# cbrl/BNN-PYNQ

Measured on AMD Instinct MI355X. Metric: images/sec (whole node) CNV-W1A1 CIFAR-10-shape batch, higher is better.
Workload: dtype u1; 1 GPU; cnvW1A1, 131072 synthetic 32x32x3 uint8 images per GPU per step, inputs resident in HBM, params cifar10/cnvW1A1; parallelism=dp1 (batch shards, no data-path collective)

## Files before the change

### bnn-pynq_amd/csrc/kernels.hip

```cpp
#include <hip/hip_runtime.h>
#include <hip/hip_ext.h>
#include <stdint.h>

#include <cstdlib>
#include <cstring>
#include <type_traits>

#define BNN_HD __host__ __device__
#include "act_faults.h"
#include "kernels.h"
#include "packed_params.h"
static_assert(bnn::kL0TileOffset == (int)bnn::kL0MfmaTileOffset && bnn::kL0BigBytes == (int)bnn::kL0MfmaBigBytes,
              "k_conv0_tile's operand offsets must be the ones packed_params.cpp writes the layer-0 table by");

namespace bnn {
namespace {

typedef const uint32_t __attribute__((address_space(4))) *kptr32;
typedef const uint64_t __attribute__((address_space(4))) *kptr64;

constexpr int kBlock = 256;
constexpr int kLfcFusedMaxA2 = 2048;

struct BlockMap { int cg, item; bool valid; };
// ... 410 lines not shown
      const uint4 v = wt[(tap * 2 + mt) * 64 + lane];
      wreg[tap][mt] = v8i{(int)v.x, (int)v.y, (int)v.z, (int)v.w, 0, 0, 0, 0};
    }
  __shared__ v16f seed_lds[2][2];
  if (tid < 64) reinterpret_cast<float *>(seed_lds)[tid] = reinterpret_cast<const float *>(tab + kL1MfmaWeights)[tid];
  const int cc = c < 28 ? c : 27;
  uint32_t pre[15];
  auto fetch = [&](int pair) {
    const int img0 = pair * 2, lim = min(2, n_images - img0) * 1800;
#pragma unroll
    for (int j = 0; j < 15; j++) {
      const int d = tid + 256 * j;
      pre[j] = d < lim ? in[(size_t)img0 * 1800 + d] : 0u;
    }
  };
  if (blockIdx.x * 2 < n_images) fetch(blockIdx.x);
  for (int pair = blockIdx.x; pair * 2 < n_images; pair += gridDim.x) {
    const int img0 = pair * 2, nimg = min(2, n_images - img0);
    __syncthreads();
#pragma unroll
    for (int j = 0; j < 15; j++) {
      const int d = tid + 256 * j;
      if (d < nimg * 1800) {
        const int i = d >= 1800, e = d - i * 1800, pix = e >> 1, hh = e & 1;
        const uint32_t bits = pre[j];
        plane[i][hh][pix] = make_uint4(lut[bits & 255], lut[(bits >> 8) & 255], lut[(bits >> 16) & 255], lut[bits >> 24]);
      }
    }
    if ((pair + gridDim.x) * 2 < n_images) fetch(pair + gridDim.x);
    __syncthreads();
    for (int rp = wave; rp < nimg * 14; rp += 4) {
      const int i = rp / 14, r = rp - i * 14;
      const uint4 *__restrict__ P = &plane[i][h][0];
      v16f acc[2][2] = {{seed_lds[0][h], seed_lds[0][h]}, {seed_lds[1][h], seed_lds[1][h]}};
#pragma unroll
      for (int kx = 0; kx < 3; kx++) {
        v8i b[4];
#pragma unroll
        for (int y = 0; y < 4; y++) {
          const uint4 v = P[(2 * r + y) * 30 + cc + kx];
          b[y] = v8i{(int)v.x, (int)v.y, (int)v.z, (int)v.w, 0, 0, 0, 0};
        }
#pragma unroll
        for (int ky = 0; ky < 3; ky++)
#pragma unroll
          for (int mt = 0; mt < 2; mt++)
#pragma unroll
            for (int pt = 0; pt < 2; pt++)
              acc[mt][pt] = __builtin_amdgcn_mfma_scale_f32_32x32x64_f8f6f4(wreg[ky * 3 + kx][mt], b[ky + pt], acc[mt][pt], 4, 4, 0,
                                                                              0x7F7F7F7F, 0, 0x7F7F7F7F);
      }
      uint32_t word[2];
#pragma unroll
      for (int mt = 0; mt < 2; mt++) {
        int v[16];
#pragma unroll
        for (int k = 0; k < 16; k++) v[k] = __float_as_int(fmaxf(acc[mt][0][k], acc[mt][1][k]));
        const uint32_t nf = or_halves(sign_nibbles(v, h));
        const uint32_t pooled = nf & (uint32_t)__builtin_amdgcn_mov_dpp((int)nf, 0xB1, 0xF, 0xF, true);
        word[mt] = ~pooled;
      }
      if (h == 0 && c < 28 && !(c & 1))
        *reinterpret_cast<uint2 *>(out + ((size_t)(img0 + i) * 196 + r * 14 + (c >> 1)) * 2) = make_uint2(word[0], word[1]);
    }
  }
}

template <int WIN, int CD, int NT, bool POOL, int G>
__global__ __launch_bounds__(256, 2) void k_conv_mfma(const uint32_t *__restrict__ in, uint32_t *__restrict__ out,
                                                       const uint8_t *__restrict__ tab, int n_images) {
  constexpr int WOUT = WIN - 2, RP = WOUT / 2, IPI = RP * WOUT, KH = CD / 2, KS = 9 * KH, STREAMS = 4 / NT;
  constexpr int PIX = WIN * WIN, DWI = PIX * CD, NPF = (G * DWI + 255) / 256;
  static_assert(WOUT % 2 == 0 && IPI % 2 == 0 && (NT == 2 || NT == 4), "tile geometry");
  __shared__ uint4 plane[G][CD][PIX];
  __shared__ uint32_t lut[256];
  const int tid = threadIdx.x, lane = tid & 63, wave = tid >> 6, mt = wave % NT, c = lane & 31, h = lane >> 5;
  lut[tid] = fp4_pm1((uint32_t)tid);
  const uint4 *__restrict__ wt = reinterpret_cast<const uint4 *>(tab);
  v8i wreg[KS];
#pragma unroll
  for (int ks = 0; ks < KS; ks++) {
    const uint4 v = wt[(ks * NT + mt) * 64 + lane];
    wreg[ks] = v8i{(int)v.x, (int)v.y, (int)v.z, (int)v.w, 0, 0, 0, 0};
  }
  const v16f seed = reinterpret_cast<const v16f *>(tab + (size_t)KS * NT * 64 * 16)[mt * 2 + h];
  const int ngroups = (n_images + G - 1) / G;
  uint32_t pre[NPF];
  auto fetch = [&](int grp) {
    const int img0 = grp * G, lim = min(G, n_images - img0) * DWI;
#pragma unroll
    for (int j = 0; j < NPF; j++) {
      const int d = tid + 256 * j;
      pre[j] = d < lim ? in[(size_t)img0 * DWI + d] : 0u;
    }
  };
  if (blockIdx.x < ngroups) fetch(blockIdx.x);
  for (int grp = blockIdx.x; grp < ngroups; grp += gridDim.x) {
    const int img0 = grp * G, nimg = min(G, n_images - img0), nitems = nimg * IPI;
    __syncthreads();
#pragma unroll
    for (int j = 0; j < NPF; j++) {
      const int d = tid + 256 * j;
      if (d < nimg * DWI) {
        const int i = d / DWI, e = d - i * DWI, pix = e / CD, q = e % CD;
        const uint32_t bits = pre[j];
        plane[i][q][pix] = make_uint4(lut[bits & 255], lut[(bits >> 8) & 255], lut[(bits >> 16) & 255], lut[bits >> 24]);
      }
    }
    if (grp + (int)gridDim.x < ngroups) fetch(grp + gridDim.x);
    __syncthreads();
    for (int t0 = (wave / NT) * 32; t0 < nitems; t0 += 32 * STREAMS) {
      const int item = min(t0 + c, nitems - 1);
      const int i = item / IPI, rem = item - i * IPI, rp = rem / WOUT, x = rem - rp * WOUT;
      v16f acc[2] = {seed, seed};
#pragma unroll
      for (int kh = 0; kh < KH; kh++) {
        const uint4 *__restrict__ P = &plane[i][kh * 2 + h][2 * rp * WIN + x];
#pragma unroll
        for (int kx = 0; kx < 3; kx++) {
          v8i b[4];
#pragma unroll
          for (int y = 0; y < 4; y++) {
            const uint4 v = P[y * WIN + kx];
            b[y] = v8i{(int)v.x, (int)v.y, (int)v.z, (int)v.w, 0, 0, 0, 0};
          }
#pragma unroll
          for (int ky = 0; ky < 3; ky++)
#pragma unroll
            for (int dy = 0; dy < 2; dy++)
              acc[dy] = __builtin_amdgcn_mfma_scale_f32_32x32x64_f8f6f4(wreg[(ky * 3 + kx) * KH + kh], b[ky + dy], acc[dy], 4, 4, 0,
                                                                         0x7F7F7F7F, 0, 0x7F7F7F7F);
        }
      }
      const bool valid = t0 + c < nitems;
      const size_t img = (size_t)(img0 + i);
      if constexpr (POOL) {
        int v[16];
#pragma unroll
        for (int k = 0; k < 16; k++) v[k] = __float_as_int(fmaxf(acc[0][k], acc[1][k]));
        const uint32_t nf = or_halves(sign_nibbles(v, h));
        const uint32_t pooled = nf & (uint32_t)__builtin_amdgcn_mov_dpp((int)nf, 0xB1, 0xF, 0xF, true);
        if (valid && h == 0 && !(x & 1)) out[(img * (RP * RP) + rp * RP + (x >> 1)) * NT + mt] = ~pooled;
      } else {
        uint32_t nf[2];
#pragma unroll
        for (int dy = 0; dy < 2; dy++) {
          int v[16];
#pragma unroll
          for (int k = 0; k < 16; k++) v[k] = __float_as_int(acc[dy][k]);
          nf[dy] = or_halves(sign_nibbles(v, h));
        }
        if (valid) out[(img * (WOUT * WOUT) + (2 * rp + h) * WOUT + x) * NT + mt] = ~(h ? nf[1] : nf[0]);
      }
    }
  }
}

__global__ __launch_bounds__(256) void k_conv_mfma_table(const uint32_t *__restrict__ rows, int row_dw, int ksteps, int tiles,
                                                          int mw, uint8_t *__restrict__ dst) {
  const int idx = blockIdx.x * 256 + threadIdx.x, nw = ksteps * tiles * 64;
  if (idx < nw) {
    const int ks = idx / (tiles * 64), mt = (idx / 64) % tiles, lane = idx & 63, n = 32 * mt + (lane & 31), h = lane >> 5;
    const uint32_t bits = rows[(size_t)n * row_dw + 2 + 2 * ks + h];
    reinterpret_cast<uint4 *>(dst)[idx] = make_uint4(fp4_pm1(bits & 255), fp4_pm1((bits >> 8) & 255), fp4_pm1((bits >> 16) & 255),
                                                     fp4_pm1(bits >> 24));
  } else if (idx < nw + tiles * 32) {
    const int j = idx - nw, mt = j >> 5, h = (j >> 4) & 1, reg = j & 15;
    const int n = 32 * mt + (reg & 3) + 8 * (reg >> 2) + 4 * h;
    long long t = (int)rows[(size_t)n * row_dw];
    t = t < -1 ? -1 : (t > mw + 2 ? mw + 2 : t);
    reinterpret_cast<float *>(dst + (size_t)nw * 16)[j] = (float)(-(mw - 2 * t) - 1);
  }
}

__device__ __forceinline__ uint32_t nibble_spread(uint32_t byte) {
  uint32_t t = byte & 0xFFu;
  t = (t | (t << 12)) & 0x000F000Fu;
  t = (t | (t << 6)) & 0x03030303u;
  return (t | (t << 3)) & 0x11111111u;
}
__device__ __forceinline__ uint4 fp4_planes(const uint32_t *lutz, const uint32_t *luts, uint32_t sg, uint32_t nz) {
  const uint32_t m = sg & nz;
  return make_uint4(lutz[nz & 255] | luts[m & 255], lutz[(nz >> 8) & 255] | luts[(m >> 8) & 255],
                    lutz[(nz >> 16) & 255] | luts[(m >> 16) & 255], lutz[nz >> 24] | luts[m >> 24]);
}
__device__ __forceinline__ void not_fired(const v16f &acc, const v16f &dt, int h, uint32_t &n0, uint32_t &n1) {
  int v[16], u[16];
#pragma unroll
  for (int k = 0; k < 16; k++) {
    v[k] = __float_as_int(acc[k]);
    u[k] = __float_as_int(acc[k] - dt[k]);
  }
  n0 = or_halves(sign_nibbles(v, h));
  n1 = or_halves(sign_nibbles(u, h));
}

template <int WIN, int CD, int NT, bool POOL, int G>
__global__ __launch_bounds__(256, 2) void k_conv_mfma_a2(const uint4 *__restrict__ in, uint32_t *__restrict__ out,
                                                          const uint8_t *__restrict__ tab, int n_images) {
  constexpr int WOUT = WIN - 2, RP = WOUT / 2, IPI = RP * WOUT, KH = CD / 2, KS = 9 * KH, STREAMS = 4 / NT;
  constexpr int PIX = WIN * WIN, QWI = PIX * KH, NPF = (G * QWI + 255) / 256;
  static_assert(WOUT % 2 == 0 && IPI % 2 == 0 && (NT == 2 || NT == 4), "tile geometry");
  __shared__ uint4 plane[G][CD][PIX];
  __shared__ uint32_t lutz[256], luts[256];
  const int tid = threadIdx.x, lane = tid & 63, wave = tid >> 6, mt = wave % NT, c = lane & 31, h = lane >> 5;
  lutz[tid] = nibble_spread((uint32_t)tid) << 1;
  luts[tid] = nibble_spread((uint32_t)tid) << 3;
  const uint4 *__restrict__ wt = reinterpret_cast<const uint4 *>(tab);
  v8i wreg[KS];
#pragma unroll
  for (int ks = 0; ks < KS; ks++) {
    const uint4 v = wt[(ks * NT + mt) * 64 + lane];
    wreg[ks] = v8i{(int)v.x, (int)v.y, (int)v.z, (int)v.w, 0, 0, 0, 0};
  }
  const v16f *__restrict__ cst = reinterpret_cast<const v16f *>(tab + (size_t)KS * NT * 64 * 16);
  const v16f seed = cst[mt * 2 + h], dt = cst[NT * 2 + mt * 2 + h];
  const int ngroups = (n_images + G - 1) / G;
  uint4 pre[NPF];
  auto fetch = [&](int grp) {
    const int img0 = grp * G, lim = min(G, n_images - img0) * QWI;
#pragma unroll
    for (int j = 0; j < NPF; j++) {
      const int d = tid + 256 * j;
      pre[j] = d < lim ? in[(size_t)img0 * QWI + d] : make_uint4(0u, 0u, 0u, 0u);
    }
  };
  if (blockIdx.x < ngroups) fetch(blockIdx.x);
  for (int grp = blockIdx.x; grp < ngroups; grp += gridDim.x) {
    const int img0 = grp * G, nimg = min(G, n_images - img0), nitems = nimg * IPI;
    __syncthreads();
#pragma unroll
    for (int j = 0; j < NPF; j++) {
      const int d = tid + 256 * j;
      if (d < nimg * QWI) {
        const int i = d / QWI, e = d - i * QWI, pix = e / KH, cw = e % KH;
        const uint4 v = pre[j];
        plane[i][2 * cw][pix] = fp4_planes(lutz, luts, v.x, v.z);
        plane[i][2 * cw + 1][pix] = fp4_planes(lutz, luts, v.y, v.w);
      }
    }
    if (grp + (int)gridDim.x < ngroups) fetch(grp + gridDim.x);
    __syncthreads();
    for (int t0 = (wave / NT) * 32; t0 < nitems; t0 += 32 * STREAMS) {
      const int item = min(t0 + c, nitems - 1);
      const int i = item / IPI, rem = item - i * IPI, rp = rem / WOUT, x = rem - rp * WOUT;
      v16f acc[2] = {seed, seed};
#pragma unroll
      for (int kh = 0; kh < KH; kh++) {
        const uint4 *__restrict__ P = &plane[i][kh * 2 + h][2 * rp * WIN + x];
#pragma unroll
        for (int kx = 0; kx < 3; kx++) {
          v8i b[4];
#pragma unroll
          for (int y = 0; y < 4; y++) {
            const uint4 v = P[y * WIN + kx];
            b[y] = v8i{(int)v.x, (int)v.y, (int)v.z, (int)v.w, 0, 0, 0, 0};
          }
#pragma unroll
          for (int ky = 0; ky < 3; ky++)
#pragma unroll
            for (int dy = 0; dy < 2; dy++)
              acc[dy] = __builtin_amdgcn_mfma_scale_f32_32x32x64_f8f6f4(wreg[(ky * 3 + kx) * KH + kh], b[ky + dy], acc[dy], 4, 4, 0,
                                                                         0x7F7F7F7F, 0, 0x7F7F7F7F);
        }
      }
      const bool valid = t0 + c < nitems;
      const size_t img = (size_t)(img0 + i);
      if constexpr (POOL) {
        v16f top;
#pragma unroll
        for (int k = 0; k < 16; k++) top[k] = fmaxf(acc[0][k], acc[1][k]);
        uint32_t n0, n1;
        not_fired(top, dt, h, n0, n1);
        n0 &= (uint32_t)__builtin_amdgcn_mov_dpp((int)n0, 0xB1, 0xF, 0xF, true);
        n1 &= (uint32_t)__builtin_amdgcn_mov_dpp((int)n1, 0xB1, 0xF, 0xF, true);
        const size_t w64 = (img * (RP * RP) + rp * RP + (x >> 1)) * (NT / 2) + mt / 2;
        if (valid && !(x & 1)) out[(w64 * 2 + h) * 2 + (mt & 1)] = h ? ~(n0 ^ n1) : (n0 & n1);
      } else {
        uint32_t n0[2], n1[2];
#pragma unroll
        for (int dy = 0; dy < 2; dy++) not_fired(acc[dy], dt, h, n0[dy], n1[dy]);
        const uint32_t m0 = h ? n0[1] : n0[0], m1 = h ? n1[1] : n1[0];
        const size_t w64 = (img * (WOUT * WOUT) + (2 * rp + h) * WOUT + x) * (NT / 2) + mt / 2;
        if (valid) {
          out[(w64 * 2 + 0) * 2 + (mt & 1)] = m0 & m1;
          out[(w64 * 2 + 1) * 2 + (mt & 1)] = ~(m0 ^ m1);
        }
      }
    }
  }
}

template <bool TT>
__global__ __launch_bounds__(256) void k_conv_mfma_a2_table(const uint32_t *__restrict__ rows, int ksteps, int tiles,
                                                             uint8_t *__restrict__ dst) {
  const int idx = blockIdx.x * 256 + threadIdx.x, nw = ksteps * tiles * 64, row_dw = TT ? 4 + 6 * ksteps : 2 + 2 * ksteps;
  if (idx < nw) {
    const int ks = idx / (tiles * 64), mt = (idx / 64) % tiles, lane = idx & 63, n = 32 * mt + (lane & 31), h = lane >> 5;
    const uint32_t *__restrict__ row = rows + (size_t)n * row_dw;
    uint32_t b1, b2 = 0, b3;
    if constexpr (TT) {
      const uint32_t sg = row[2 + 4 * ks + h], two = row[2 + 4 * ksteps + 2 * ks + h], nz = row[2 + 4 * ks + 2 + h] | two;
      b1 = nz & ~two;
      b2 = two;
      b3 = (sg & nz) | two;
    } else {
// ... 1265 lines not shown
  const int32_t *__restrict__ c = classes + (size_t)q * n;
  long long at = 0;
  if constexpr (EMIT) {
    if (counts[q] == 0) return;
    at = offsets[q];
  }
  int total = 0;
  for (int j0 = 0; j0 < win; j0 += kBlock) {
    const int j = j0 + tid;
    const int32_t v = j < win ? c[j] : 0;
    const bool ch = j < win && v != base[j];
    if constexpr (EMIT) {
      const uint64_t m = __ballot(ch);
      if (lane == 0) wave_n[wave] = __popcll(m);
      __syncthreads();
      int before = 0, all = 0;
      for (int w = 0; w < kBlock / 64; w++) {
        before += w < wave ? wave_n[w] : 0;
        all += wave_n[w];
      }
      if (ch) {
        const long long o = at + before + __popcll(m & ((1ull << lane) - 1));
        out[2 * o] = j;
        out[2 * o + 1] = v;
      }
      at += all;
      __syncthreads();
    } else {
      total += __syncthreads_count(ch);
    }
  }
  if constexpr (!EMIT) {
    if (tid == 0) counts[q] = total;
  }
}

template <bool TWO_BIT>
__global__ __launch_bounds__(kBlock) void k_act_seed(const uint8_t *__restrict__ base, uint8_t *__restrict__ act, int row_units,
                                                     const MultiSeg *__restrict__ segs, const ActPatch *__restrict__ patches, int per_seg,
                                                     long long units) {
  const long long t = (long long)blockIdx.x * kBlock + threadIdx.x;
  if (t >= units) return;
  const long long q = t / per_seg;
  const int r = (int)(t - q * per_seg), j = r / row_units, u = r - j * row_units;
  const MultiSeg sg = segs[q];
  if (j >= sg.len) return;
  uint4 v = reinterpret_cast<const uint4 *>(base)[(size_t)(sg.image + j) * row_units + u];
  const ActPatch p = patches[sg.run];
  if (u == (int)p.unit) {
    const uint32_t m = 1u << (p.bit & 31), h = p.bit >> 5;
    if constexpr (!TWO_BIT) {
      v.x ^= h == 0 ? m : 0u;
      v.y ^= h == 1 ? m : 0u;
      v.z ^= h == 2 ? m : 0u;
      v.w ^= h == 3 ? m : 0u;
    } else {
      uint32_t sgn = h ? v.y : v.x, nz = h ? v.w : v.z;
      const uint32_t i = (sgn & m) ? 0u : ((nz & m) ? 2u : 1u), k = (i + p.shift) % 3u;
      sgn = k == 0 ? (sgn | m) : (sgn & ~m);
      nz = k != 1 ? (nz | m) : (nz & ~m);
      if (h) { v.y = sgn; v.w = nz; } else { v.x = sgn; v.z = nz; }
    }
  }
  reinterpret_cast<uint4 *>(act)[(size_t)(sg.slot + j) * row_units + u] = v;
}

template <bool TWO_BIT>
__global__ __launch_bounds__(kBlock) void k_act_noise(uint32_t *__restrict__ act, unsigned row_words, const MultiSeg *__restrict__ segs,
                                                      const unsigned long long *__restrict__ seeds, unsigned layer, unsigned rate,
                                                      unsigned long long *__restrict__ counts, unsigned nlayers) {
  const MultiSeg sg = segs[blockIdx.y];
  const unsigned t = blockIdx.x * kBlock + threadIdx.x;
  uint32_t fired = 0;
  if (t < (unsigned)sg.len * row_words) {
    const unsigned j = t / row_words, w = t - j * row_words;
    const unsigned long long seed = seeds[sg.run];
    const uint32_t k0 = (uint32_t)seed, k1 = (uint32_t)(seed >> 32), image = (uint32_t)sg.image + j;
    uint32_t two = 0;
#pragma unroll
    for (int b = 0; b < 8; b++) {
      uint32_t u[4];
      act_noise_block(k0, k1, image, layer, w * 8 + b, u);
#pragma unroll
      for (int e = 0; e < 4; e++) {
        const uint32_t f = u[e] < rate ? 1u : 0u;
        fired |= f << (4 * b + e);
        if constexpr (TWO_BIT) two |= (f & u[e]) << (4 * b + e);
      }
    }
    if (fired) {
      const size_t row = (size_t)(sg.slot + j) * row_words;
      if constexpr (!TWO_BIT) {
        act[row + w] ^= fired;
      } else {
        uint32_t *const p = act + 2 * row + (size_t)(w >> 1) * 4 + (w & 1);
        const uint32_t sgn = p[0], nz = p[2], one = fired & ~two;
        const uint32_t i0 = sgn, i1 = ~sgn & ~nz, i2 = ~sgn & nz;
        const uint32_t n0 = (i2 & one) | (i1 & two), n1 = (i0 & one) | (i2 & two);
        p[0] = (sgn & ~fired) | n0;
        p[2] = (nz & ~fired) | (fired & ~n1);
      }
    }
  }
  unsigned c = __popc(fired);
#pragma unroll
  for (int d = 32; d >= 1; d >>= 1) c += __shfl_xor(c, d, 64);
  if ((threadIdx.x & 63) == 0 && c) atomicAdd(counts + (size_t)sg.run * nlayers + layer, (unsigned long long)c);
}

inline long long lfc_fused_max() {
  static const long long v = [] {
    const char *e = std::getenv("BNN_MI355X_LFC_FUSED_MAX");
    return e ? std::atoll(e) : 1024LL;
  }();
  return v;
}
inline long long lfc_block_max() {
  static const long long v = [] {
    const char *e = std::getenv("BNN_MI355X_LFC_BLOCK_MAX");
    return e ? std::atoll(e) : 131072LL;
  }();
  return v;
}

inline long long l0_tile_min() {
  static const long long v = [] {
    const char *e = std::getenv("BNN_MI355X_L0_TILE_MIN");
    return e ? std::atoll(e) : 8192LL;
  }();
  return v;
}

constexpr long long kConvMfmaMinW1A2 = 384, kConvMfmaMinW2A2 = 256;
inline long long conv_mfma_min() {
  static const long long v = [] {
    const char *e = std::getenv("BNN_MI355X_CONV_MFMA_MIN");
    return e ? std::atoll(e) : 512LL;
  }();
  return v;
}
template <int ARITH>
inline long long conv_mfma_a2_min() {
  static const long long v = [] {
    const char *e = std::getenv("BNN_MI355X_CONV_MFMA_MIN");
    return e ? std::atoll(e) : (ARITH == AR_TT ? kConvMfmaMinW2A2 : kConvMfmaMinW1A2);
  }();
  return v;
}
template <int ARITH, bool OUT2>
inline const uint8_t *conv_mfma_for(const CnvLaunch &a) {
  if constexpr (ARITH == AR_XNOR && !OUT2) return a.n >= conv_mfma_min() ? a.conv_mfma : nullptr;
  else return a.n >= conv_mfma_a2_min<ARITH>() ? a.conv_mfma : nullptr;
}
constexpr long long kTailMfmaMinW1A1 = 3072, kTailMfmaMinW1A2 = 3072, kTailMfmaMinW2A2 = 1024;
constexpr int kTailMfmaStages = 0xF0;
template <int ARITH>
inline long long tail_mfma_min() {
  static const long long v = [] {
    const char *e = std::getenv("BNN_MI355X_TAIL_MFMA_MIN");
    return e ? std::atoll(e) : (ARITH == AR_XNOR ? kTailMfmaMinW1A1 : ARITH == AR_TB ? kTailMfmaMinW1A2 : kTailMfmaMinW2A2);
  }();
  return v;
}
template <int ARITH>
inline const uint8_t *tail_mfma_for(const CnvLaunch &a) {
  if (a.done_flag && a.n == 1) return nullptr;
  return a.n >= tail_mfma_min<ARITH>() ? a.conv_mfma : nullptr;
}
inline unsigned persistent_grid(long long units, long long cap) {
  const long long per = (units + cap - 1) / cap;
  return (unsigned)((units + per - 1) / per);
}
constexpr long long kConvMfmaGrid = 512;
constexpr int kConvMfmaImgsL1 = 2, kConvMfmaImgs = 8;
constexpr int kTailMfmaImgsL4 = 32, kTailMfmaImgsL5 = 32, kTailMfmaImgsFc = 128;
constexpr long long kTailMfmaGrid8 = 256;
#define BNN_TAIL_MFMA(A2, KS, NT, CONV, WAVES, G, cap, in, out, tab)                                                               \
  hipLaunchKernelGGL((k_tail_mfma<A2, KS, NT, CONV, WAVES, G>), dim3(persistent_grid((n + (G) - 1) / (G), (cap))), dim3(64 * (WAVES)), 0, s, \
                     in, out, tab, (int)n)

inline int gpb_for(long long items, int groups) { return (items + kBlock - 1) / kBlock >= 2048 ? groups : 1; }

inline bool narrow_for(long long items, int groups32, long long limit) { return ((items + kBlock - 1) / kBlock) * groups32 < limit; }
constexpr long long kNarrowLimitCnv = 8192, kNarrowLimitLfc = 512;
constexpr long long kFcLastWaveMax = 32768;
constexpr long long kPixelLaneMax = 512;
constexpr long long kCnvTailMax = 1024;

inline dim3 grid_for(long long items, int groups) {
  const long long item_blocks = (items + kBlock - 1) / kBlock;
  return dim3((unsigned)(((item_blocks + 7) / 8) * 8 * groups));
}

#define BNN_LAUNCH(kern, grid, stream, ...)                                   \
  do {                                                                        \
    if ((grid).x > 0) hipLaunchKernelGGL(kern, grid, dim3(kBlock), 0, stream, __VA_ARGS__); \
  } while (0)
#define BNN_STAGE(kern32, kern8, items, groups32, in, out, rows)                                                                   \
  do {                                                                                                                             \
    const long long it_ = (items);                                                                                                 \
    if (narrow_for(it_, (groups32), narrow_limit)) BNN_LAUNCH(kern8, grid_for(it_, (groups32) * 4), s, in, out, rows, (int)it_, (groups32) * 4, 1); \
    else BNN_LAUNCH(kern32, grid_for(it_, (groups32) / gpb_for(it_, (groups32))), s, in, out, rows, (int)it_, (groups32), gpb_for(it_, (groups32))); \
  } while (0)
#define BNN_MARK(ev, i, stream)                          \
  do {                                                   \
    if (ev) (void)hipEventRecord((ev)[i], stream);       \
  } while (0)

template <int ARITH, bool OUT2, bool TWO = false>
void run_cnv_t(const CnvLaunch &a) {
  const long long n = a.n, narrow_limit = kNarrowLimitCnv;
  uint32_t *A = reinterpret_cast<uint32_t *>(a.buf0), *B = reinterpret_cast<uint32_t *>(a.buf1);
  const uint64_t *A64 = reinterpret_cast<const uint64_t *>(a.buf0), *B64 = reinterpret_cast<const uint64_t *>(a.buf1);
  hipStream_t s = a.stream;
  BNN_MARK(a.events, 0, s);
  if (a.l0_mfma) {
    const dim3 g0((unsigned)((n * 900 + kBlock - 1) / kBlock));
    if (a.last_stage >= 0) {
      if (n >= l0_tile_min()) BNN_LAUNCH((k_conv0_tile<OUT2>), dim3((unsigned)((n + kL0Imgs - 1) / kL0Imgs)), s, a.images, A, a.l0_mfma, (int)n);
      else BNN_LAUNCH((k_conv0_mfma<OUT2>), g0, s, a.images, A, a.l0_mfma, (int)(n * 900));
    }
  } else {
    if (a.last_stage >= 0) BNN_LAUNCH((k_conv0<OUT2>), grid_for(n * 900, 2 / gpb_for(n * 900, 2)), s, a.images, A, a.rows[0], (int)(n * 900), 2, gpb_for(n * 900, 2));
  }
  BNN_MARK(a.events, 1, s);
  if constexpr (ARITH == AR_XNOR && !OUT2) {
    const bool pix = n <= kPixelLaneMax;
    const uint8_t *const cm = conv_mfma_for<ARITH, OUT2>(a);
    const dim3 g1(persistent_grid((n + kConvMfmaImgsL1 - 1) / kConvMfmaImgsL1, kConvMfmaGrid)),
        gm(persistent_grid((n + kConvMfmaImgs - 1) / kConvMfmaImgs, kConvMfmaGrid));
    if (a.last_stage >= 1) {
      if (a.l1_literal) {
        BNN_LAUNCH(k_l1_literal, dim3((unsigned)((n * 784 + kBlock - 1) / kBlock)), s, A64, reinterpret_cast<uint64_t *>(B), a.rows[1], (int)(n * 784));
      } else if (a.l1_mfma) {
        const long long pairs = (n + 1) / 2;
        hipLaunchKernelGGL(k_l1_mfma, dim3((unsigned)(pairs < 512 ? pairs : 512)), dim3(256), 0, s, reinterpret_cast<const uint32_t *>(a.buf0), B,
                           a.l1_mfma, (int)n);
      } else if (cm) {
        hipLaunchKernelGGL((k_conv_mfma<30, 2, 2, true, kConvMfmaImgsL1>), g1, dim3(256), 0, s, reinterpret_cast<const uint32_t *>(a.buf0), B, cm,
                           (int)n);
      } else if (pix) BNN_LAUNCH((k_vec_x<9, true, 1, 30, 8, true>), grid_for(n * 784, 8), s, A64, B, a.rows[1], (int)(n * 784), 8, 1);
      else BNN_STAGE((k_quad_x<1, 30, true>), (k_quad_x<1, 30, true, 8>), n * 196, 2, A64, B, a.rows[1]);
    }
    BNN_MARK(a.events, 2, s);
    if (a.last_stage >= 2) {
      if (cm) hipLaunchKernelGGL((k_conv_mfma<14, 2, 4, false, kConvMfmaImgs>), gm, dim3(256), 0, s, B, A, cm + kConvMfmaL2Off, (int)n);
      else if (pix) BNN_LAUNCH((k_vec_x<9, true, 1, 14, 8>), grid_for(n * 144, 16), s, B64, A, a.rows[2], (int)(n * 144), 16, 1);
      else BNN_STAGE((k_quad_x<1, 14, false>), (k_quad_x<1, 14, false, 8>), n * 36, 4, B64, A, a.rows[2]);
    }
    BNN_MARK(a.events, 3, s);
    if (a.last_stage >= 3) {
      if (cm) hipLaunchKernelGGL((k_conv_mfma<12, 4, 4, true, kConvMfmaImgs>), gm, dim3(256), 0, s, A, B, cm + kConvMfmaL3Off, (int)n);
      else if (pix) BNN_LAUNCH((k_vec_x<18, true, 2, 12, 8, true>), grid_for(n * 100, 16), s, A64, B, a.rows[3], (int)(n * 100), 16, 1);
      else BNN_STAGE((k_quad_x<2, 12, true>), (k_quad_x<2, 12, true, 8>), n * 25, 4, A64, B, a.rows[3]);
    }
    BNN_MARK(a.events, 4, s);
    const uint8_t *const tm = tail_mfma_for<ARITH>(a);
    const uint32_t *const A32 = A, *const B32 = B;
    if (!tm && n <= kCnvTailMax && !a.events && a.last_stage >= kCnvStages - 1) {
      hipLaunchKernelGGL(k_cnv_tail, dim3((unsigned)n), dim3(512), 0, s, B64, a.scores, a.classes, a.rows[4], a.rows[5], a.rows[6],
                         a.rows[7], a.rows[8], a.number_class, n == 1 ? a.done_flag : nullptr, a.done_seq);
      return;
    }
    if (a.last_stage >= 4) {
      if (tm && (kTailMfmaStages & 16)) BNN_TAIL_MFMA(false, 18, 8, true, 8, kTailMfmaImgsL4, kTailMfmaGrid8, B32, A, tm + kTailMfmaL4Off);
      else BNN_STAGE((k_vec_x<18, true, 2, 5>), (k_vec_x<18, true, 2, 5, 8>), n * 9, 8, B64, A, a.rows[4]);
    }
    BNN_MARK(a.events, 5, s);
    if (a.last_stage >= 5) {
      if (tm && (kTailMfmaStages & 32)) BNN_TAIL_MFMA(false, 36, 8, false, 8, kTailMfmaImgsL5, kTailMfmaGrid8, A32, B, tm + kTailMfmaL5Off);
      else BNN_STAGE((k_vec_x<36, false, 1, 1>), (k_vec_x<36, false, 1, 1, 8>), n, 8, A64, B, a.rows[5]);
    }
    BNN_MARK(a.events, 6, s);
    if (a.last_stage >= 6) {
      if (tm && (kTailMfmaStages & 64)) BNN_TAIL_MFMA(false, 4, 16, false, 4, kTailMfmaImgsFc, kConvMfmaGrid, B32, A, tm + kTailMfmaL6Off);
      else BNN_STAGE((k_vec_x<4, false, 1, 1>), (k_vec_x<4, false, 1, 1, 8>), n, 16, B64, A, a.rows[6]);
    }
    BNN_MARK(a.events, 7, s);
    if (a.last_stage >= 7) {
      if (tm && (kTailMfmaStages & 128)) BNN_TAIL_MFMA(false, 8, 16, false, 8, kTailMfmaImgsFc, kTailMfmaGrid8, A32, B, tm + kTailMfmaL7Off);
      else BNN_STAGE((k_vec_x<8, false, 1, 1>), (k_vec_x<8, false, 1, 1, 8>), n, 16, A64, B, a.rows[7]);
    }
    BNN_MARK(a.events, 8, s);
  } else {
    const bool pix = n <= kPixelLaneMax;
    const uint8_t *const cm = conv_mfma_for<ARITH, OUT2>(a);
    const uint4 *const A128 = reinterpret_cast<const uint4 *>(a.buf0), *const B128 = reinterpret_cast<const uint4 *>(a.buf1);
    const dim3 g1(persistent_grid((n + kConvMfmaImgsL1 - 1) / kConvMfmaImgsL1, kConvMfmaGrid)),
        gm(persistent_grid((n + kConvMfmaImgs - 1) / kConvMfmaImgs, kConvMfmaGrid));
    if (a.last_stage >= 1) {
      if (cm) hipLaunchKernelGGL((k_conv_mfma_a2<30, 2, 2, true, kConvMfmaImgsL1>), g1, dim3(256), 0, s, A128, B, cm, (int)n);
      else if (pix) BNN_LAUNCH((k_vec<ARITH, 9, OUT2, true, 1, 30, 8, true, TWO>), grid_for(n * 784, 8), s, A64, B, a.rows[1], (int)(n * 784), 8, 1);
      else BNN_STAGE((k_quad<ARITH, 1, 30, true, OUT2, 32, TWO>), (k_quad<ARITH, 1, 30, true, OUT2, 8, TWO>), n * 196, 2, A64, B, a.rows[1]);
    }
    BNN_MARK(a.events, 2, s);
    if (a.last_stage >= 2) {
      if (cm) hipLaunchKernelGGL((k_conv_mfma_a2<14, 2, 4, false, kConvMfmaImgs>), gm, dim3(256), 0, s, B128, A, cm + kConvMfmaA2L2Off, (int)n);
      else if (pix) BNN_LAUNCH((k_vec<ARITH, 9, OUT2, true, 1, 14, 8, false, TWO>), grid_for(n * 144, 16), s, B64, A, a.rows[2], (int)(n * 144), 16, 1);
      else BNN_STAGE((k_quad<ARITH, 1, 14, false, OUT2, 32, TWO>), (k_quad<ARITH, 1, 14, false, OUT2, 8, TWO>), n * 36, 4, B64, A, a.rows[2]);
    }
    BNN_MARK(a.events, 3, s);
    if (a.last_stage >= 3) {
      if (cm) hipLaunchKernelGGL((k_conv_mfma_a2<12, 4, 4, true, kConvMfmaImgs>), gm, dim3(256), 0, s, A128, B, cm + kConvMfmaA2L3Off, (int)n);
      else if (pix) BNN_LAUNCH((k_vec<ARITH, 18, OUT2, true, 2, 12, 8, true, TWO>), grid_for(n * 100, 16), s, A64, B, a.rows[3], (int)(n * 100), 16, 1);
      else BNN_STAGE((k_quad<ARITH, 2, 12, true, OUT2, 32, TWO>), (k_quad<ARITH, 2, 12, true, OUT2, 8, TWO>), n * 25, 4, A64, B, a.rows[3]);
    }
    BNN_MARK(a.events, 4, s);
    const uint8_t *const tm = tail_mfma_for<ARITH>(a);
    if constexpr (!TWO) {
      if (!tm && n <= kCnvTailMax && !a.events && a.last_stage >= kCnvStages - 1) {
        hipLaunchKernelGGL((k_cnv_tail_a2<ARITH>), dim3((unsigned)n), dim3(512), 0, s, B64, a.scores, a.classes, a.rows[4], a.rows[5],
                           a.rows[6], a.rows[7], a.rows[8], a.number_class, n == 1 ? a.done_flag : nullptr, a.done_seq);
        return;
      }
    }
    if (a.last_stage >= 4) {
      if (tm && (kTailMfmaStages & 16)) BNN_TAIL_MFMA(true, 18, 8, true, 8, kTailMfmaImgsL4, kTailMfmaGrid8, B128, A, tm + kTailMfmaA2L4Off);
      else BNN_STAGE((k_vec<ARITH, 18, OUT2, true, 2, 5, 32, false, TWO>), (k_vec<ARITH, 18, OUT2, true, 2, 5, 8, false, TWO>), n * 9, 8, B64, A, a.rows[4]);
    }
    BNN_MARK(a.events, 5, s);
    if (a.last_stage >= 5) {
      if (tm && (kTailMfmaStages & 32)) BNN_TAIL_MFMA(true, 36, 8, false, 8, kTailMfmaImgsL5, kTailMfmaGrid8, A128, B, tm + kTailMfmaA2L5Off);
      else BNN_STAGE((k_vec<ARITH, 36, OUT2, false, 1, 1, 32, false, TWO>), (k_vec<ARITH, 36, OUT2, false, 1, 1, 8, false, TWO>), n, 8, A64, B, a.rows[5]);
    }
    BNN_MARK(a.events, 6, s);
    if (a.last_stage >= 6) {
      if (tm && (kTailMfmaStages & 64)) BNN_TAIL_MFMA(true, 4, 16, false, 4, kTailMfmaImgsFc, kConvMfmaGrid, B128, A, tm + kTailMfmaA2L6Off);
      else BNN_STAGE((k_vec<ARITH, 4, OUT2, false, 1, 1, 32, false, TWO>), (k_vec<ARITH, 4, OUT2, false, 1, 1, 8, false, TWO>), n, 16, B64, A, a.rows[6]);
    }
    BNN_MARK(a.events, 7, s);
    if (a.last_stage >= 7) {
      if (tm && (kTailMfmaStages & 128)) BNN_TAIL_MFMA(true, 8, 16, false, 8, kTailMfmaImgsFc, kTailMfmaGrid8, A128, B, tm + kTailMfmaA2L7Off);
      else BNN_STAGE((k_vec<ARITH, 8, OUT2, false, 1, 1, 32, false, TWO>), (k_vec<ARITH, 8, OUT2, false, 1, 1, 8, false, TWO>), n, 16, A64, B, a.rows[7]);
    }
    BNN_MARK(a.events, 8, s);
  }
  if (a.last_stage >= 8) {
    if (n <= kFcLastWaveMax) BNN_LAUNCH((k_fclast_wave<ARITH, 8, TWO>), dim3((unsigned)((n + 3) / 4)), s, B64, a.scores, a.classes, a.rows[8], (int)n, a.number_class);
    else BNN_LAUNCH((k_fclast<ARITH, 8, TWO>), grid_for(n, 1), s, B64, a.scores, a.classes, a.rows[8], (int)n, a.number_class);
  }
  BNN_MARK(a.events, 9, s);
}

template <int ARITH, bool OUT2>
int matrix_stages_t(const CnvLaunch &a) {
  const bool cm = conv_mfma_for<ARITH, OUT2>(a) != nullptr;
  bool l1 = cm;
  if constexpr (ARITH == AR_XNOR && !OUT2) l1 = !a.l1_literal && (a.l1_mfma || cm);
  return (a.l0_mfma ? 1 : 0) | (l1 ? 2 : 0) | (cm ? 12 : 0) | (tail_mfma_for<ARITH>(a) ? kTailMfmaStages : 0);
}

#define BNN_MULTI(kern, ipi, groups32, in, out, rows, RES)                                                               \
  do {                                                                                                                   \
    const long long it_ = (long long)a.total * (ipi);                                                                    \
    const int gpb_ = gpb_for(it_, (groups32));                                                                           \
    const MultiArgs ma_{a.segs, (unsigned)(a.stride / 4), (ipi), (RES) ? a.n : 0};                                       \
    dim3 g_ = grid_for((long long)a.max_len * (ipi), (groups32) / gpb_);                                                 \
    g_.y = (unsigned)a.nsegs;                                                                                            \
    BNN_LAUNCH(kern, g_, s, in, out, rows, (int)it_, (groups32), gpb_, ma_);                                             \
  } while (0)

template <int ARITH, bool OUT2, bool TWO = false>
void run_cnv_multi_t(const MultiLaunch &a) {
  uint32_t *A = reinterpret_cast<uint32_t *>(a.buf0), *B = reinterpret_cast<uint32_t *>(a.buf1);
  const uint64_t *A64 = reinterpret_cast<const uint64_t *>(a.buf0), *B64 = reinterpret_cast<const uint64_t *>(a.buf1);
  hipStream_t s = a.stream;
  const auto in = [&](int l) { return a.first <= l && l <= a.last; };
  if (in(0) && a.l0_mfma) {
    const MultiArgs ma{a.segs, (unsigned)(a.stride / 4), 1, 0};
    BNN_LAUNCH((k_conv0_tile<OUT2, true>), dim3((unsigned)((a.max_len + kL0Imgs - 1) / kL0Imgs), (unsigned)a.nsegs), s, a.images, A,
               a.l0_mfma, 0, ma);
  } else if (in(0)) {
    BNN_MULTI((k_conv0<OUT2, true>), 900, 2, a.images, A, a.rows[0], false);
  }
  if constexpr (ARITH == AR_XNOR && !OUT2) {
    if (in(1)) BNN_MULTI((k_quad_x<1, 30, true, 32, true>), 196, 2, A64, B, a.rows[1], false);
    if (in(2)) BNN_MULTI((k_quad_x<1, 14, false, 32, true>), 36, 4, B64, A, a.rows[2], false);
    if (in(3)) BNN_MULTI((k_quad_x<2, 12, true, 32, true>), 25, 4, A64, B, a.rows[3], false);
    if (in(4)) BNN_MULTI((k_vec_x<18, true, 2, 5, 32, false, true>), 9, 8, B64, A, a.rows[4], false);
    if (in(5)) BNN_MULTI((k_vec_x<36, false, 1, 1, 32, false, true>), 1, 8, A64, B, a.rows[5], false);
    if (in(6)) BNN_MULTI((k_vec_x<4, false, 1, 1, 32, false, true>), 1, 16, B64, A, a.rows[6], false);
    if (in(7)) BNN_MULTI((k_vec_x<8, false, 1, 1, 32, false, true>), 1, 16, A64, B, a.rows[7], false);
  } else {
    if (in(1)) BNN_MULTI((k_quad<ARITH, 1, 30, true, OUT2, 32, TWO, true>), 196, 2, A64, B, a.rows[1], false);
    if (in(2)) BNN_MULTI((k_quad<ARITH, 1, 14, false, OUT2, 32, TWO, true>), 36, 4, B64, A, a.rows[2], false);
    if (in(3)) BNN_MULTI((k_quad<ARITH, 2, 12, true, OUT2, 32, TWO, true>), 25, 4, A64, B, a.rows[3], false);
    if (in(4)) BNN_MULTI((k_vec<ARITH, 18, OUT2, true, 2, 5, 32, false, TWO, true>), 9, 8, B64, A, a.rows[4], false);
    if (in(5)) BNN_MULTI((k_vec<ARITH, 36, OUT2, false, 1, 1, 32, false, TWO, true>), 1, 8, A64, B, a.rows[5], false);
    if (in(6)) BNN_MULTI((k_vec<ARITH, 4, OUT2, false, 1, 1, 32, false, TWO, true>), 1, 16, B64, A, a.rows[6], false);
    if (in(7)) BNN_MULTI((k_vec<ARITH, 8, OUT2, false, 1, 1, 32, false, TWO, true>), 1, 16, A64, B, a.rows[7], false);
// ... 320 lines not shown
```

Baseline: 36.34 million images/s.

## Add software-pipelined conv1 MFMA kernel with register prefetch and preloaded weights

Adds a new layer-1 convolution kernel that holds all nine weight k-steps in registers, prefetches the next image group from global memory into registers while the current group is expanded into shared memory, and double-buffers the shared-memory operand reads across output tiles. It also replaces the float max for pooling with a bitwise AND of the sign bits. The path is used when the batch is at least 512 and the l1_literal and l1_mfma paths are not taken. It aims to hide global and LDS latency, at the cost of higher register pressure under launch_bounds(256,2).

```diff
diff --git a/bnn-pynq_amd/csrc/kernels.hip b/bnn-pynq_amd/csrc/kernels.hip
--- a/bnn-pynq_amd/csrc/kernels.hip
+++ b/bnn-pynq_amd/csrc/kernels.hip
@@ -586,6 +586,102 @@
         }
         if (valid) out[(img * (WOUT * WOUT) + (2 * rp + h) * WOUT + x) * NT + mt] = ~(h ? nf[1] : nf[0]);
       }
+    }
+  }
+}
+
+template <int WIN, int NT, int G>
+__global__ __launch_bounds__(256, 2) void k_conv_mfma_pipe(const uint32_t *__restrict__ in, uint32_t *__restrict__ out,
+                                                            const uint8_t *__restrict__ tab, int n_images) {
+  constexpr int CD = 2, WOUT = WIN - 2, RP = WOUT / 2, IPI = RP * WOUT, KS = 9, STREAMS = 4 / NT, STRIDE = 32 * STREAMS;
+  constexpr int PIX = WIN * WIN, DWI = PIX * CD, NPF = (G * DWI + 255) / 256;
+  static_assert(WOUT % 2 == 0 && IPI % 2 == 0 && (NT == 2 || NT == 4), "tile geometry");
+  __shared__ uint4 plane[G][CD][PIX];
+  __shared__ uint32_t lut[256];
+  const int tid = threadIdx.x, lane = tid & 63, wave = tid >> 6, mt = wave % NT, c = lane & 31, h = lane >> 5;
+  lut[tid] = fp4_pm1((uint32_t)tid);
+  const uint4 *__restrict__ wt = reinterpret_cast<const uint4 *>(tab);
+  v8i wreg[KS];
+#pragma unroll
+  for (int ks = 0; ks < KS; ks++) {
+    const uint4 v = wt[(ks * NT + mt) * 64 + lane];
+    wreg[ks] = v8i{(int)v.x, (int)v.y, (int)v.z, (int)v.w, 0, 0, 0, 0};
+  }
+  const v16f seed = reinterpret_cast<const v16f *>(tab + (size_t)KS * NT * 64 * 16)[mt * 2 + h];
+  const int ngroups = (n_images + G - 1) / G;
+  uint32_t pre[NPF];
+  auto fetch = [&](int grp) {
+    const int img0 = grp * G, lim = min(G, n_images - img0) * DWI;
+#pragma unroll
+    for (int j = 0; j < NPF; j++) {
+      const int d = tid + 256 * j;
+      pre[j] = d < lim ? in[(size_t)img0 * DWI + d] : 0u;
+    }
+  };
+  if (blockIdx.x < ngroups) fetch(blockIdx.x);
+  for (int grp = blockIdx.x; grp < ngroups; grp += gridDim.x) {
+    const int img0 = grp * G, nimg = min(G, n_images - img0), nitems = nimg * IPI;
+    __syncthreads();
+#pragma unroll
+    for (int j = 0; j < NPF; j++) {
+      const int d = tid + 256 * j;
+      if (d < nimg * DWI) {
+        const int i = d / DWI, e = d - i * DWI, pix = e / CD, q = e % CD;
+        const uint32_t bits = pre[j];
+        plane[i][q][pix] = make_uint4(lut[bits & 255], lut[(bits >> 8) & 255], lut[(bits >> 16) & 255], lut[bits >> 24]);
+      }
+    }
+    if (grp + (int)gridDim.x < ngroups) fetch(grp + gridDim.x);
+    __syncthreads();
+    const int first = (wave / NT) * 32;
+    if (first >= nitems) continue;
+    const int ntw = (nitems - first + STRIDE - 1) / STRIDE;
+    constexpr uint32_t kNowhere = 0xFFFFFFFFu;
+    auto locate = [&](int t0, const uint4 *&corner, uint32_t &oidx) {
+      const int item = min(t0 + c, nitems - 1);
+      const int i = item / IPI, rem = item - i * IPI, rp = rem / WOUT, x = rem - rp * WOUT;
+      corner = &plane[i][h][2 * rp * WIN + x];
+      const uint32_t o = ((uint32_t)(img0 + i) * (RP * RP) + rp * RP + (x >> 1)) * NT + mt;
+      oidx = t0 + c < nitems && h == 0 && !(x & 1) ? o : kNowhere;
+    };
+    v4i b[3][4];
+    auto rd = [&](const uint4 *corner) {
+#pragma unroll
+      for (int kx = 0; kx < 3; kx++)
+#pragma unroll
+        for (int y = 0; y < 4; y++) {
+          const uint4 v = corner[y * WIN + kx];
+          b[kx][y] = v4i{(int)v.x, (int)v.y, (int)v.z, (int)v.w};
+        }
+    };
+    const uint4 *corner_c;
+    uint32_t oidx_c;
+    locate(first, corner_c, oidx_c);
+    rd(corner_c);
+    for (int k = 0; k < ntw; k++) {
+      const uint4 *corner_n;
+      uint32_t oidx_n;
+      locate(first + (k + 1) * STRIDE, corner_n, oidx_n);
+      v16f acc[2] = {seed, seed};
+#pragma unroll
+      for (int kx = 0; kx < 3; kx++)
+#pragma unroll
+        for (int ky = 0; ky < 3; ky++)
+#pragma unroll
+          for (int dy = 0; dy < 2; dy++) {
+            const v4i o = b[kx][ky + dy];
+            acc[dy] = __builtin_amdgcn_mfma_scale_f32_32x32x64_f8f6f4(wreg[ky * 3 + kx], v8i{o.x, o.y, o.z, o.w, 0, 0, 0, 0}, acc[dy], 4, 4, 0,
+                                                                       0x7F7F7F7F, 0, 0x7F7F7F7F);
+          }
+      rd(corner_n);
+      int v[16];
+#pragma unroll
+      for (int r = 0; r < 16; r++) v[r] = __float_as_int(acc[0][r]) & __float_as_int(acc[1][r]);
+      const uint32_t nf = or_halves(sign_nibbles(v, h));
+      const uint32_t pooled = nf & (uint32_t)__builtin_amdgcn_mov_dpp((int)nf, 0xB1, 0xF, 0xF, true);
+      if (oidx_c != kNowhere) out[oidx_c] = ~pooled;
+      corner_c = corner_n;
+      oidx_c = oidx_n;
     }
   }
 }
@@ -2157,6 +2253,14 @@
   if constexpr (ARITH == AR_XNOR && !OUT2) return a.n >= conv_mfma_min() ? a.conv_mfma : nullptr;
   else return a.n >= conv_mfma_a2_min<ARITH>() ? a.conv_mfma : nullptr;
 }
+constexpr long long kConvPipeMin = 512;
+inline long long conv_pipe_min() {
+  static const long long v = [] {
+    const char *e = std::getenv("BNN_MI355X_CONV_PIPE_MIN");
+    return e ? std::atoll(e) : kConvPipeMin;
+  }();
+  return v;
+}
 constexpr long long kTailMfmaMinW1A1 = 3072, kTailMfmaMinW1A2 = 3072, kTailMfmaMinW2A2 = 1024;
 constexpr int kTailMfmaStages = 0xF0;
 template <int ARITH>
@@ -2232,6 +2336,7 @@
   if constexpr (ARITH == AR_XNOR && !OUT2) {
     const bool pix = n <= kPixelLaneMax;
     const uint8_t *const cm = conv_mfma_for<ARITH, OUT2>(a);
+    const bool pipe = n >= conv_pipe_min();
     const dim3 g1(persistent_grid((n + kConvMfmaImgsL1 - 1) / kConvMfmaImgsL1, kConvMfmaGrid)),
         gm(persistent_grid((n + kConvMfmaImgs - 1) / kConvMfmaImgs, kConvMfmaGrid));
     if (a.last_stage >= 1) {
@@ -2241,6 +2346,9 @@
         const long long pairs = (n + 1) / 2;
         hipLaunchKernelGGL(k_l1_mfma, dim3((unsigned)(pairs < 512 ? pairs : 512)), dim3(256), 0, s, reinterpret_cast<const uint32_t *>(a.buf0), B,
                            a.l1_mfma, (int)n);
+      } else if (cm && pipe) {
+        hipLaunchKernelGGL((k_conv_mfma_pipe<30, 2, kConvMfmaImgsL1>), g1, dim3(256), 0, s, reinterpret_cast<const uint32_t *>(a.buf0),
+                           B, cm, (int)n);
       } else if (cm) {
         hipLaunchKernelGGL((k_conv_mfma<30, 2, 2, true, kConvMfmaImgsL1>), g1, dim3(256), 0, s, reinterpret_cast<const uint32_t *>(a.buf0), B, cm,
                            (int)n);
```

After: 38.75 million images/s (median of 6 runs). 6.6% higher.
